# callmeray/PointMVSNet

Hardware: NVIDIA H100
Metric: PointFlow iters/sec (higher is better)
Workload: dtype f32

## Files before the change

### include/pmvs_b200.h

```cpp
#ifndef PMVS_B200_H_
#define PMVS_B200_H_

#include <stddef.h>
#include <stdint.h>

#ifdef __cplusplus
extern "C" {
#endif

#define PMVS_OK 0
#define PMVS_ERR_ARG 1
#define PMVS_ERR_CUDA 2
#define PMVS_ERR_WORKSPACE 3

#define PMVS_NUM_HYP 5
#define PMVS_FEAT_CH 136
#define PMVS_KNN 16
#define PMVS_MAX_VIEWS 12

typedef void* pmvs_stream_t;

int pmvs_version(void);
const char* pmvs_last_error(void);
unsigned long long pmvs_launch_count(void);

int pmvs_set_gemm_mode(int mode);
int pmvs_get_gemm_mode(void);

#define PMVS_OPT_EDGE 1
#define PMVS_OPT_KNN 2
#define PMVS_OPT_FETCH 3
#define PMVS_OPT_GEMM 4
#define PMVS_OPT_DEBUG_IDX 5
int pmvs_set_option(int key, int value);
int pmvs_get_option(int key);

int pmvs_profile_enable(int on);
int pmvs_profile_collect(char* names, size_t names_bytes, float* ms, int max_records);

int pmvs_gather_knn_forward(const float* input, const int64_t* index, float* output,
                            int B, int C, int N, int K, pmvs_stream_t stream);
int pmvs_gather_knn_backward(const float* grad_output, const int64_t* index, float* grad_input,
                             int B, int C, int N, int K, pmvs_stream_t stream);
size_t pmvs_gather_knn_backward_det_workspace_bytes(int B, int N, int K);
int pmvs_gather_knn_backward_det(const float* grad_output, const int64_t* index, float* grad_input,
                                 int B, int C, int N, int K, void* workspace, size_t workspace_bytes,
                                 pmvs_stream_t stream);

int pmvs_knn3d(const float* xyz, int64_t* idx64, int32_t* idx32, int B, int D, int H, int W,
               int ksize, int knn, pmvs_stream_t stream);

int pmvs_feature_fetch(const float* feature_maps, const float* pts, const float* intrinsics,
                       const float* extrinsics, float* out, int B, int V, int C, int H, int W,
                       int N, pmvs_stream_t stream);
int pmvs_feature_fetch_backward(const float* grad_out, const float* pts, const float* intrinsics,
                                const float* extrinsics, float* grad_maps, int B, int V, int C,
                                int H, int W, int N, pmvs_stream_t stream);

int pmvs_cost_volume(const float* features, const float* cam_params, float* cost, void* workspace,
                     size_t workspace_bytes, int B, int V, int C, int h, int w, int D, int is_test,
                     pmvs_stream_t stream);

int pmvs_transpose(const float* in, float* out, int batch, int R, int C, pmvs_stream_t stream);
int pmvs_idx64_to_idx32(const int64_t* in, int32_t* out, long long n, pmvs_stream_t stream);

int pmvs_edgeconv_pm(const float* x, int ldx, const int32_t* idx32, const float* w12,
                     const float* gamma, const float* beta, float eps, int concat_central,
                     int bn_train, float* out, int ldo, float* le_scratch, double* stats_scratch,
                     int groups, int rows_per_group, int N, int K, int cin, int cout,
                     pmvs_stream_t stream);

int pmvs_linear_pm(const float* x, int ldx, const float* w, float* y, int ldy, int groups,
                   int rows_per_group, int cin, int cout, const double* in_stats,
                   const float* in_gamma, const float* in_beta, double in_count, float eps,
                   double* out_stats, pmvs_stream_t stream);

typedef struct pmvs_flow_weights {
  const float* ec_w12[3];
  const float* ec_gamma[3];
  const float* ec_beta[3];
  const float* mlp_w[4];
  const float* mlp_gamma[3];
  const float* mlp_beta[3];
  float* ec_run_mean[3];
  float* ec_run_var[3];
  float* mlp_run_mean[3];
// ... 38 lines not shown
```

### pointmvsnet_b200/_lib.py

```python
import ctypes as C
import os

import torch

_HERE = os.path.dirname(os.path.abspath(__file__))
LIB_PATH = os.path.join(_HERE, "libpmvs_b200.so")

if not os.path.exists(LIB_PATH):
    raise ImportError(
        "pointmvsnet_b200: %s is missing -- build it with pointmvsnet_b200/csrc/build.sh "
        "(nvcc, sm_90a).  There is no CPU fallback." % LIB_PATH)

lib = C.CDLL(LIB_PATH)

c_float_p = C.c_void_p
c_stream = C.c_void_p


class FlowWeights(C.Structure):
    _fields_ = [
        ("ec_w12", C.c_void_p * 3), ("ec_gamma", C.c_void_p * 3), ("ec_beta", C.c_void_p * 3),
        ("mlp_w", C.c_void_p * 4), ("mlp_gamma", C.c_void_p * 3), ("mlp_beta", C.c_void_p * 3),
        ("ec_run_mean", C.c_void_p * 3), ("ec_run_var", C.c_void_p * 3),
        ("mlp_run_mean", C.c_void_p * 3), ("mlp_run_var", C.c_void_p * 3),
# ... 49 lines not shown
EXPORTED = [
    "pmvs_version", "pmvs_last_error", "pmvs_launch_count", "pmvs_set_option", "pmvs_get_option", "pmvs_profile_enable", "pmvs_profile_collect", "pmvs_set_gemm_mode", "pmvs_get_gemm_mode", "pmvs_gather_knn_forward",
    "pmvs_gather_knn_backward", "pmvs_gather_knn_backward_det_workspace_bytes", "pmvs_gather_knn_backward_det", "pmvs_knn3d", "pmvs_feature_fetch", "pmvs_feature_fetch_backward",
    "pmvs_cost_volume", "pmvs_transpose", "pmvs_idx64_to_idx32", "pmvs_edgeconv_pm", "pmvs_linear_pm", "pmvs_point_flow_workspace_bytes",
    "pmvs_point_flow_iter", "pmvs_pyramid_to_channels_last", "pmvs_point_flow_debug_offsets",
]


def check(rc):
    if rc != 0:
        raise RuntimeError("libpmvs_b200: " + lib.pmvs_last_error().decode("utf-8", "replace"))


def stream_ptr():
    return torch.cuda.current_stream().cuda_stream


def ptr(t):
    return None if t is None else t.data_ptr()


def require_cuda(*tensors):
    for t in tensors:
        if t is not None and not t.is_cuda:
            raise RuntimeError("pointmvsnet_b200 operators need CUDA tensors (sm_90a); there is no CPU fallback")


def f32c(t):
    if t.dtype != torch.float32:
        t = t.float()
    return t.contiguous()


def launch_count():
    return int(lib.pmvs_launch_count())


def profile_enable(on):
    lib.pmvs_profile_enable(1 if on else 0)


def profile_collect(max_records=65536):
    names = C.create_string_buffer(max_records * 24)
    ms = (C.c_float * max_records)()
    n = lib.pmvs_profile_collect(names, len(names), C.cast(ms, C.c_void_p), max_records)
    nm = names.value.decode().split("\n")[:n]
    return [(nm[i], float(ms[i])) for i in range(n)]


def set_gemm_mode(mode):
    check(lib.pmvs_set_gemm_mode(int(mode)))


OPTIONS = {"edge": 1, "knn": 2, "fetch": 3, "gemm": 4, "debug_idx": 5}


def set_option(name, value):
    check(lib.pmvs_set_option(OPTIONS[name], int(value)))


def get_option(name):
    return int(lib.pmvs_get_option(OPTIONS[name]))


def _options_from_env():
    spec = os.environ.get("PMVS_OPTIONS", "")
    for item in spec.split(","):
        if "=" in item:
            k, v = item.split("=", 1)
            set_option(k.strip(), int(v))


_options_from_env()
```

### pointmvsnet_b200/csrc/api.cu

```cuda
#include <algorithm>
#include <atomic>
#include <cstdarg>
#include <mutex>
#include <vector>

#include "common.cuh"

namespace pmvs {

static thread_local char g_err[512] = "";
static std::atomic<unsigned long long> g_launches{0};

void set_error(const char* fmt, ...) {
  va_list ap;
  va_start(ap, fmt);
  vsnprintf(g_err, sizeof(g_err), fmt, ap);
  va_end(ap);
}
void count_launch(int n) { g_launches.fetch_add((unsigned long long)n, std::memory_order_relaxed); }

static std::atomic<int> g_opt[OPT_COUNT];
static struct OptDefaults {
  OptDefaults() {
    g_opt[OPT_EDGE].store(1);
    g_opt[OPT_KNN].store(1);
    g_opt[OPT_FETCH].store(1);
    g_opt[OPT_GEMM].store(2);
  }
} g_opt_defaults;
int opt(int key) { return (key >= 0 && key < OPT_COUNT) ? g_opt[key].load(std::memory_order_relaxed) : 0; }

struct ProfRec {
  const char* name;
  cudaEvent_t a, b;
};
static std::mutex g_prof_mu;
static std::vector<ProfRec> g_prof;
static std::atomic<int> g_prof_on{0};
static thread_local int g_prof_open = -1;

void prof_begin(const char* what, cudaStream_t st) {
  if (!g_prof_on.load(std::memory_order_relaxed)) return;
  ProfRec r;
  r.name = what;
  if (cudaEventCreate(&r.a) != cudaSuccess || cudaEventCreate(&r.b) != cudaSuccess) return;
  cudaEventRecord(r.a, st);
  std::lock_guard<std::mutex> lk(g_prof_mu);
  g_prof.push_back(r);
  g_prof_open = (int)g_prof.size() - 1;
}
void prof_end(cudaStream_t st) {
  if (g_prof_open < 0) return;
  std::lock_guard<std::mutex> lk(g_prof_mu);
  if (g_prof_open < (int)g_prof.size()) cudaEventRecord(g_prof[g_prof_open].b, st);
  g_prof_open = -1;
}

__global__ void __launch_bounds__(256) transpose_kernel(const float* __restrict__ in, float* __restrict__ out, int R,
                                                        int C) {
  __shared__ float tile[32][33];
  const size_t boff = (size_t)blockIdx.z * R * C;
  const int c0 = blockIdx.x * 32, r0 = blockIdx.y * 32;
  const int tx = threadIdx.x & 31, ty = threadIdx.x >> 5;
#pragma unroll
  for (int j = 0; j < 32; j += 8) {
    const int r = r0 + ty + j, c = c0 + tx;
    if (r < R && c < C) tile[ty + j][tx] = __ldg(in + boff + (size_t)r * C + c);
  }
  __syncthreads();
#pragma unroll
  for (int j = 0; j < 32; j += 8) {
    const int c = c0 + ty + j, r = r0 + tx;
    if (r < R && c < C) out[boff + (size_t)c * R + r] = tile[tx][ty + j];
  }
}

int launch_transpose(const float* in, float* out, int batch, int R, int C, cudaStream_t st) {
  PMVS_REQUIRE(in && out && batch > 0 && R > 0 && C > 0, "transpose: bad arguments");
  PMVS_REQUIRE(batch <= 65535 && cdiv(R, 32) <= 65535, "transpose: shape too large");
  dim3 grid(cdiv(C, 32), cdiv(R, 32), batch);
// ... 393 lines not shown
```

### pointmvsnet_b200/csrc/common.cuh

```cuda
#pragma once
#include <cuda_runtime.h>
#include <stdint.h>
#include <stdio.h>
#include <string.h>

#include "../../include/pmvs_b200.h"

namespace pmvs {

void set_error(const char* fmt, ...);
void count_launch(int n = 1);

void prof_begin(const char* what, cudaStream_t st);
void prof_end(cudaStream_t st);

inline int check_launch(const char* what, cudaStream_t st = nullptr) {
  cudaError_t e = cudaPeekAtLastError();
  if (e != cudaSuccess) {
    cudaGetLastError();
    set_error("%s: %s", what, cudaGetErrorString(e));
    return PMVS_ERR_CUDA;
  }
  prof_end(st);
  count_launch();
  return PMVS_OK;
}

#define PMVS_REQUIRE(cond, ...)     \
  do {                              \
    if (!(cond)) {                  \
      pmvs::set_error(__VA_ARGS__); \
      return PMVS_ERR_ARG;          \
    }                               \
  } while (0)

#define PMVS_TRY(expr)           \
  do {                           \
    int _rc = (expr);            \
    if (_rc != PMVS_OK) return _rc; \
  } while (0)

static inline int cdiv(long long a, long long b) { return (int)((a + b - 1) / b); }

inline int sm_count() {
  static int n = 0;
  if (n == 0) {
    int dev = 0, v = 0;
    cudaGetDevice(&dev);
    n = (cudaDeviceGetAttribute(&v, cudaDevAttrMultiProcessorCount, dev) == cudaSuccess && v > 0) ? v : 132;
  }
  return n;
}

__device__ __forceinline__ float4 ldg4(const float* p) { return __ldg(reinterpret_cast<const float4*>(p)); }
__device__ __forceinline__ void st4(float* p, float4 v) { *reinterpret_cast<float4*>(p) = v; }

typedef float2 f32x2;
__device__ __forceinline__ f32x2 pack2(float a, float b) { return make_float2(a, b); }
__device__ __forceinline__ void unpack2(f32x2 v, float& a, float& b) { a = v.x; b = v.y; }
__device__ __forceinline__ f32x2 fma2(f32x2 a, f32x2 b, f32x2 c) { return make_float2(__fmaf_rn(a.x, b.x, c.x), __fmaf_rn(a.y, b.y, c.y)); }
__device__ __forceinline__ f32x2 add2(f32x2 a, f32x2 b) { return make_float2(__fadd_rn(a.x, b.x), __fadd_rn(a.y, b.y)); }
__device__ __forceinline__ f32x2 mul2(f32x2 a, f32x2 b) { return make_float2(__fmul_rn(a.x, b.x), __fmul_rn(a.y, b.y)); }
__device__ __forceinline__ f32x2 sub2(f32x2 a, f32x2 b) { return make_float2(__fsub_rn(a.x, b.x), __fsub_rn(a.y, b.y)); }

enum {
  OPT_EDGE = 1,
  OPT_KNN = 2,
  OPT_FETCH = 3,
  OPT_GEMM = 4,
  OPT_DEBUG_IDX = 5,
  OPT_COUNT = 16
};
int opt(int key);

template <typename K>
inline int ensure_dyn_smem(K kernel, int bytes, unsigned long long& done_mask, const char* what) {
  int dev = 0;
  if (cudaGetDevice(&dev) != cudaSuccess || dev < 0 || dev > 63) dev = 0;
  if (done_mask & (1ull << dev)) return PMVS_OK;
  if (cudaFuncSetAttribute(kernel, cudaFuncAttributeMaxDynamicSharedMemorySize, bytes) != cudaSuccess) {
    cudaGetLastError();
    set_error("%s: cannot reserve %d bytes of shared memory", what, bytes);
    return PMVS_ERR_CUDA;
  }
  done_mask |= 1ull << dev;
  return PMVS_OK;
}

struct BnCoef {
  float mean, invstd;
};
__device__ __forceinline__ BnCoef bn_coef(double s1, double s2, double count, float eps) {
  double m = s1 / count;
  double var = s2 / count - m * m;
  if (var < 0.0) var = 0.0;
  BnCoef c;
  c.mean = (float)m;
  c.invstd = (float)(1.0 / sqrt(var + (double)eps));
  return c;
}
__device__ __forceinline__ float bn_apply(float x, float mean, float invstd, float g, float b) {
  return __fadd_rn(__fmul_rn(__fmul_rn(__fsub_rn(x, mean), invstd), g), b);
}

int launch_knn3d_cand(const float* xyz, int32_t* idx32, unsigned short* cand, int clouds, int D, int H, int W,
                      cudaStream_t st);
int launch_knn3d(const float* xyz, int64_t* idx64, int32_t* idx32, int clouds, int D, int H, int W,
                 int ksize, int knn, cudaStream_t st);
int launch_transpose(const float* in, float* out, int batch, int R, int C, cudaStream_t st);

struct GemmArgs {
  const float* x;
  int ldx;
  const float* w;
  float* y;
  int ldy;
  int groups, rows_per_group, cin, cout;
  const double* in_stats;
  const float* in_gamma;
  const float* in_beta;
  double in_count;
  float eps;
  double* out_stats;
// ... 90 lines not shown
```

### pointmvsnet_b200/csrc/edge_tile.cu

```cuda
#include <algorithm>
#include <cuda.h>

#include "common.cuh"

namespace pmvs {

namespace {

constexpr int ET_THREADS = 256;
constexpr int ET_WARPS = ET_THREADS / 32;
constexpr int ET_CP = 32;
constexpr int ET_LPP = ET_CP / 4;
constexpr int ET_PPW = 32 / ET_LPP;

typedef CUresult (*EncodeTiledFn)(CUtensorMap*, CUtensorMapDataType, cuuint32_t, void*, const cuuint64_t*,
                                  const cuuint64_t*, const cuuint32_t*, const cuuint32_t*, CUtensorMapInterleave,
                                  CUtensorMapSwizzle, CUtensorMapL2promotion, CUtensorMapFloatOOBfill);

EncodeTiledFn encode_fn() {
  static EncodeTiledFn fn = [] {
    void* p = nullptr;
    cudaDriverEntryPointQueryResult q;
    if (cudaGetDriverEntryPoint("cuTensorMapEncodeTiled", &p, cudaEnableDefault, &q) != cudaSuccess ||
        q != cudaDriverEntryPointSuccess)
      p = nullptr;
    cudaGetLastError();
    return (EncodeTiledFn)p;
  }();
  return fn;
}

__device__ __forceinline__ unsigned smem_u32(const void* p) { return (unsigned)__cvta_generic_to_shared(p); }

template <int TX, int TY>
struct TileGeom {
  static constexpr int HX = TX + 4, HY = TY + 4;
  static constexpr int ROWS = PMVS_NUM_HYP * HY * HX;
  static constexpr int NPTS = PMVS_NUM_HYP * TY * TX;
  static constexpr int BYTES = ROWS * ET_CP * 4;
  static constexpr int SMEM = BYTES;
};

constexpr int ET_COEF = 6;

template <int COUT, bool APPLY, int TX, int TY>
__global__ void __launch_bounds__(ET_THREADS, 3) edge_tile_kernel(const __grid_constant__ CUtensorMap tm,
                                                                   const EdgeTileArgs a) {
  using G = TileGeom<TX, TY>;
  static_assert(COUT % ET_CP == 0, "edge_tile: channels must be a multiple of 32");
  static_assert(G::NPTS % (ET_WARPS * ET_PPW) == 0, "edge_tile: every thread owns NPTS / 32 points");
  constexpr int LD = 2 * COUT;
  constexpr int SLABS = COUT / ET_CP;
  constexpr int STEPS = G::NPTS / (ET_WARPS * ET_PPW);
  static_assert(G::HX == 12 && G::HY == 8, "the kNN kernel's 16-bit codes are row offsets of a 12 x 8 x 5 halo tile");
  extern __shared__ __align__(128) float halo[];
  __shared__ __align__(8) unsigned long long bar;
  __shared__ float part[APPLY ? 1 : ET_WARPS][APPLY ? 1 : 2 * ET_CP];
  __shared__ __align__(16) float coef[APPLY ? ET_COEF * COUT : 4];
  __shared__ int s_last;

  const int g = blockIdx.z;
  const int tid = threadIdx.x, warp = tid >> 5, lane = tid & 31;
  const int sub = lane / ET_LPP, cl = (lane % ET_LPP) * 4;
  const int gh = a.gh, gw = a.gw;
  const int tiles_x = (gw + TX - 1) / TX, tiles_per_cloud = tiles_x * ((gh + TY - 1) / TY);
  const int tiles_per_group = tiles_per_cloud * a.clouds_per_group;
  const int HW = gh * gw, N = PMVS_NUM_HYP * HW;
  const int rows_per_group = a.clouds_per_group * N;
  const unsigned bar_addr = smem_u32(&bar);

  if (tid == 0) {
    asm volatile("mbarrier.init.shared::cta.b64 [%0], 1;" ::"r"(bar_addr));
    asm volatile("fence.mbarrier_init.release.cluster;" ::: "memory");
  }
  if (APPLY) {
    const float* cg = a.coef + (size_t)g * ET_COEF * COUT;
    for (int c = tid; c < ET_COEF * COUT; c += ET_THREADS) coef[c] = __ldg(cg + c);
  }
  static_assert(TX * TY == ET_WARPS * ET_PPW && STEPS == PMVS_NUM_HYP, "edge_tile: one layer of the tile per step");
  const int tq = warp * ET_PPW + sub, tx = tq % TX, ty = tq / TX;
  const int pb0 = ((-2 * G::HY + ty) * G::HX + tx) * ET_CP + cl;
  constexpr int LAYER = G::HY * G::HX * ET_CP;
  __syncthreads();
// ... 138 lines not shown
      unpack2(n2_lo, v[4], v[5]); unpack2(n2_hi, v[6], v[7]);
#pragma unroll
      for (int off = ET_LPP; off < 32; off <<= 1) {
#pragma unroll
        for (int q = 0; q < 8; ++q) v[q] += __shfl_xor_sync(0xffffffffu, v[q], off);
      }
      if (sub == 0) {
#pragma unroll
        for (int q = 0; q < 8; ++q) part[warp][(q >> 2) * ET_CP + cl + (q & 3)] = v[q];
      }
      __syncthreads();
      double* o = a.nstats + (size_t)g * 2 * COUT;
      if (tid < 2 * ET_CP) {
        double t = 0.0;
#pragma unroll
        for (int wq = 0; wq < ET_WARPS; ++wq) t += (double)part[wq][tid];
        atomicAdd(o + (tid / ET_CP) * COUT + ch0 + (tid % ET_CP), t);
      }
    }
  }

  if (!APPLY) {
    __threadfence();
    __syncthreads();
    if (tid == 0) {
      const unsigned t = atomicAdd(a.ticket + g, 1u);
      s_last = t == gridDim.x - 1;
    }
    __syncthreads();
    if (s_last) {
      __threadfence();
      const double* sc = a.cstats + (size_t)g * 4 * COUT;
      const double* sn = a.nstats + (size_t)g * 2 * COUT;
      float* cg = a.coef + (size_t)g * ET_COEF * COUT;
      const double cnt_c = (double)rows_per_group, cnt_n = (double)rows_per_group * PMVS_KNN;
      for (int c = tid; c < COUT; c += ET_THREADS) {
        const BnCoef kn = bn_coef(__ldcg(sn + c), __ldcg(sn + COUT + c), cnt_n, a.eps);
        const int gn = a.concat_central ? COUT + c : c;
        const float A = kn.invstd * a.gamma[gn];
        cg[c] = A;
        cg[COUT + c] = fmaf(-kn.mean, A, a.beta[gn]);
        if (a.concat_central) {
          const BnCoef kc = bn_coef(sc[c], sc[2 * COUT + c], cnt_c, a.eps);
          cg[2 * COUT + c] = kc.mean; cg[3 * COUT + c] = kc.invstd; cg[4 * COUT + c] = a.gamma[c]; cg[5 * COUT + c] = a.beta[c];
        }
      }
    }
  }
}

template <int COUT, bool APPLY, int TX, int TY>
int launch_variant(const EdgeTileArgs& a, cudaStream_t st) {
  using G = TileGeom<TX, TY>;
  EncodeTiledFn enc = encode_fn();
  if (enc == nullptr) {
    set_error("edge_tile: cuTensorMapEncodeTiled is not available from this driver");
    return PMVS_ERR_CUDA;
  }
  const int N = PMVS_NUM_HYP * a.gh * a.gw;
  const long long layers = (long long)a.groups * a.clouds_per_group * PMVS_NUM_HYP;
  PMVS_REQUIRE(a.groups <= 65535 && a.clouds_per_group <= 65535, "edge_tile: too many clouds");
  PMVS_REQUIRE(layers < (1ll << 31) && (long long)a.groups * a.clouds_per_group * N < (1ll << 40), "edge_tile: too large");
  PMVS_REQUIRE(((uintptr_t)a.le & 15) == 0, "edge_tile: LE must be 16-byte aligned");
  CUtensorMap tm;
  const cuuint64_t gdim[4] = {(cuuint64_t)(2 * COUT), (cuuint64_t)a.gw, (cuuint64_t)a.gh, (cuuint64_t)layers};
  const cuuint64_t gstr[3] = {(cuuint64_t)(2 * COUT) * 4, (cuuint64_t)a.gw * 2 * COUT * 4,
                              (cuuint64_t)a.gh * a.gw * 2 * COUT * 4};
  const cuuint32_t box[4] = {ET_CP, (cuuint32_t)G::HX, (cuuint32_t)G::HY, PMVS_NUM_HYP};
  const cuuint32_t estr[4] = {1, 1, 1, 1};
  const CUresult r = enc(&tm, CU_TENSOR_MAP_DATA_TYPE_FLOAT32, 4, const_cast<float*>(a.le), gdim, gstr, box, estr,
                         CU_TENSOR_MAP_INTERLEAVE_NONE, CU_TENSOR_MAP_SWIZZLE_NONE, CU_TENSOR_MAP_L2_PROMOTION_L2_128B,
                         CU_TENSOR_MAP_FLOAT_OOB_FILL_NONE);
  if (r != CUDA_SUCCESS) {
    set_error("edge_tile: cuTensorMapEncodeTiled failed (%d) for %dx%d, cout %d", (int)r, a.gh, a.gw, COUT);
    return PMVS_ERR_CUDA;
  }
  static unsigned long long smem_done = 0;
  PMVS_TRY(ensure_dyn_smem(edge_tile_kernel<COUT, APPLY, TX, TY>, G::SMEM, smem_done, "edge_tile"));
  static int slots = 0;
  if (slots == 0) {
    slots = 3 * sm_count();
  }
  const int tiles_per_group = cdiv(a.gw, TX) * cdiv(a.gh, TY) * a.clouds_per_group;
  int ctas = APPLY ? tiles_per_group : std::min(tiles_per_group, std::max(1, slots / a.groups));
  ctas = cdiv(tiles_per_group, cdiv(tiles_per_group, ctas));
  PMVS_REQUIRE(ctas <= 0x7fffffff / 2, "edge_tile: too many tiles");
  dim3 grid(ctas, 1, a.groups);
  static const char* const names[2][2] = {{"edge_stats_32", "edge_stats_64"}, {"edge_apply_32", "edge_apply_64"}};
  prof_begin(names[APPLY ? 1 : 0][COUT == 32 ? 0 : 1], st);
  edge_tile_kernel<COUT, APPLY, TX, TY><<<grid, ET_THREADS, G::SMEM, st>>>(tm, a);
  return check_launch(APPLY ? "edge_tile_apply_kernel" : "edge_tile_stats_kernel", st);
}

template <bool APPLY>
int launch_edge_tile(const EdgeTileArgs& a, int tile_w, cudaStream_t st) {
  PMVS_REQUIRE(a.le && a.cand && a.cstats && a.nstats && a.gamma && a.beta && a.coef && a.ticket && (!APPLY || a.out),
               "edge_tile: NULL pointer");
  PMVS_REQUIRE(a.cout == 32 || a.cout == 64, "edge_tile: out_channels %d (supported: 32, 64)", a.cout);
  PMVS_REQUIRE(a.gh > 0 && a.gw > 0 && a.groups > 0 && a.clouds_per_group > 0, "edge_tile: bad cloud shape");
  (void)tile_w;
  return a.cout == 32 ? launch_variant<32, APPLY, 8, 4>(a, st) : launch_variant<64, APPLY, 8, 4>(a, st);
}

}

int launch_edge_tile_stats(const EdgeTileArgs& a, int tile_w, cudaStream_t st) {
  return launch_edge_tile<false>(a, tile_w, st);
// ... 7 lines not shown
```

### pointmvsnet_b200/csrc/gemm_ws.cu

```cuda
#include <algorithm>

#include "common.cuh"
#include "wgmma.cuh"

namespace pmvs {

namespace ws {

using namespace wg;

constexpr int NT = 128;
constexpr int KC = 32;
constexpr int PLANE_BYTES = NT * KC * 4;
constexpr int STAGE_BYTES = 2 * PLANE_BYTES;
constexpr int CONS_WARPS = 8, CONS_THREADS = CONS_WARPS * 32;
constexpr int PROD_WARPS = 8, PROD_WARP0 = CONS_WARPS, PROD_THREADS = PROD_WARPS * 32;
constexpr int THREADS = CONS_THREADS + PROD_THREADS;
constexpr int A_LD = NT * 8 / PROD_THREADS;
static_assert(A_LD * PROD_THREADS == NT * 8, "the producers share a chunk evenly");
constexpr int MAXK = 224;
constexpr int SMEM_MAX = 227 * 1024;

template <int ASYNC, int NSTAGES>
struct Layout {
  static constexpr int NST = NSTAGES;
  static constexpr int RING = 0;
  static constexpr int STAGING = RING + NST * STAGE_BYTES;
  static constexpr int W = STAGING + ASYNC * PLANE_BYTES;
};
__host__ __device__ constexpr int weight_bytes(int cout, int nch) { return nch * 2 * cout * 128; }
constexpr int TAIL_BN = 0, TAIL_RED = TAIL_BN + 2 * MAXK * 4;
__host__ __device__ constexpr int tail_bar(int cout) { return TAIL_RED + 2 * cout * 8; }
__host__ __device__ constexpr int tail_bytes(int cout) { return tail_bar(cout) + 128; }

__device__ __forceinline__ void sts128(uint32_t addr, float4 v) {
  asm volatile("st.shared.v4.f32 [%0], {%1, %2, %3, %4};" ::"r"(addr), "f"(v.x), "f"(v.y), "f"(v.z), "f"(v.w) : "memory");
}
__device__ __forceinline__ float4 lds128(uint32_t addr) {
  float4 v;
  asm volatile("ld.shared.v4.f32 {%0, %1, %2, %3}, [%4];" : "=f"(v.x), "=f"(v.y), "=f"(v.z), "=f"(v.w) : "r"(addr) : "memory");
  return v;
}
__device__ __forceinline__ float tf32_hi(float x) { return __uint_as_float(__float_as_uint(x) & 0xFFFFE000u); }

struct TileRange {
  int first, count;
};
__device__ __forceinline__ TileRange my_tiles(int total) {
  const long long G = gridDim.x, b = blockIdx.x;
  const int lo = (int)(b * total / G), hi = (int)((b + 1) * total / G);
  return TileRange{lo, hi - lo};
}

template <int COUT, bool IN_BN, int ASYNC, int NSTAGES>
__global__ void __launch_bounds__(THREADS, 1) gemm_ws_kernel(const GemmArgs a) {
// ... 247 lines not shown
          if (!ok1) v[2] = v[3] = 0.f;
          float s[4] = {v[0] + v[2], v[1] + v[3], fmaf(v[0], v[0], v[2] * v[2]), fmaf(v[1], v[1], v[3] * v[3])};
#pragma unroll
          for (int e = 0; e < 4; ++e) {
            s[e] += __shfl_xor_sync(0xffffffffu, s[e], 4);
            s[e] += __shfl_xor_sync(0xffffffffu, s[e], 8);
            s[e] += __shfl_xor_sync(0xffffffffu, s[e], 16);
          }
          if (lane < 4) {
            atomicAdd(&sRed[8 * i + fcol], (double)s[0]);
            atomicAdd(&sRed[8 * i + fcol + 1], (double)s[1]);
            atomicAdd(&sRed[COUT + 8 * i + fcol], (double)s[2]);
            atomicAdd(&sRed[COUT + 8 * i + fcol + 1], (double)s[3]);
          }
        }
      }
      if (a.out_stats != nullptr) {
        named_bar_sync(2, CONS_THREADS);
        if (tid < 2 * COUT) {
          racc += sRed[tid];
          sRed[tid] = 0.0;
        }
        named_bar_sync(2, CONS_THREADS);
      }
    }
    flush();
  }
}

constexpr int DEEP_K = 160;
template <int ASYNC, int NSTAGES>
constexpr int smem_bytes(int cout, int cin) {
  return Layout<ASYNC, NSTAGES>::W + weight_bytes(cout, (cin + KC - 1) / KC) + tail_bytes(cout);
}
constexpr bool fits(int cin, int cout) {
  return cin <= DEEP_K ? (smem_bytes<4, 2>(cout, cin) <= SMEM_MAX && smem_bytes<0, 4>(cout, cin) <= SMEM_MAX)
                       : (smem_bytes<3, 2>(cout, cin) <= SMEM_MAX && smem_bytes<0, 3>(cout, cin) <= SMEM_MAX);
}
static_assert(fits(136, 64) && fits(32, 64) && fits(64, 128) && fits(224, 64) && fits(64, 64) && fits(64, 16),
              "a hot-path GEMM shape no longer fits the shared memory of gemm_ws_kernel");

template <int COUT, bool IN_BN, int ASYNC, int NSTAGES>
static int launch_pf(const GemmArgs& a, cudaStream_t st, const char* name) {
  const int smem_total = smem_bytes<ASYNC, NSTAGES>(COUT, a.cin);
  if (smem_total > SMEM_MAX) return -1;
  static unsigned long long smem_done = 0;
  PMVS_TRY((ensure_dyn_smem(gemm_ws_kernel<COUT, IN_BN, ASYNC, NSTAGES>, SMEM_MAX, smem_done, "gemm_ws")));
  const long long tiles = (long long)a.groups * cdiv(a.rows_per_group, NT);
  const int grid = (int)std::min<long long>(tiles, sm_count());
  prof_begin(name, st);
  gemm_ws_kernel<COUT, IN_BN, ASYNC, NSTAGES><<<grid, THREADS, smem_total, st>>>(a);
  return check_launch("gemm_ws_kernel", st);
}
template <int COUT, bool IN_BN>
static int launch_one(const GemmArgs& a, cudaStream_t st, const char* name) {
  const bool deep = a.cin <= DEEP_K;
  if (opt(OPT_GEMM) == 1)
    return deep ? launch_pf<COUT, IN_BN, 0, 4>(a, st, name) : launch_pf<COUT, IN_BN, 0, 3>(a, st, name);
  return deep ? launch_pf<COUT, IN_BN, 4, 2>(a, st, name) : launch_pf<COUT, IN_BN, 3, 2>(a, st, name);
}

}

int launch_gemm_ws(const GemmArgs& a, cudaStream_t st, const char* name) {
  if (a.cin % 8 != 0 || a.cin > ws::MAXK || a.ldx % 4 != 0 || a.ldy % 2 != 0 || a.groups <= 0 || a.rows_per_group <= 0) return -1;
  if (((uintptr_t)a.x & 15) || ((uintptr_t)a.w & 15) || ((uintptr_t)a.y & 7)) return -1;
  if ((long long)a.groups * cdiv(a.rows_per_group, ws::NT) >= (1ll << 31) / ws::MAXK) return -1;
  const bool bn = a.in_stats != nullptr;
  switch (a.cout) {
    case 16: return bn ? ws::launch_one<16, true>(a, st, name) : ws::launch_one<16, false>(a, st, name);
    case 32: return bn ? ws::launch_one<32, true>(a, st, name) : ws::launch_one<32, false>(a, st, name);
    case 64: return bn ? ws::launch_one<64, true>(a, st, name) : ws::launch_one<64, false>(a, st, name);
    case 128: return bn ? ws::launch_one<128, true>(a, st, name) : ws::launch_one<128, false>(a, st, name);
  }
  return -1;
}

}
```

### pointmvsnet_b200/csrc/wgmma.cuh

```cuda
#pragma once
#include <stdint.h>

namespace pmvs {
namespace wg {

__device__ __forceinline__ uint32_t smem_u32(const void* p) { return (uint32_t)__cvta_generic_to_shared(p); }
__device__ __forceinline__ void mbar_init(uint32_t bar, uint32_t count) {
  asm volatile("mbarrier.init.shared::cta.b64 [%0], %1;" ::"r"(bar), "r"(count));
}
__device__ __forceinline__ void mbar_wait(uint32_t bar, uint32_t parity) {
  uint32_t done = 0;
  while (!done) {
    asm volatile(
        "{\n\t.reg .pred p;\n\t"
        "mbarrier.try_wait.parity.shared::cta.b64 p, [%1], %2;\n\t"
        "selp.u32 %0, 1, 0, p;\n\t}"
        : "=r"(done)
        : "r"(bar), "r"(parity)
        : "memory");
  }
}
__device__ __forceinline__ void mbar_arrive(uint32_t bar) {
  asm volatile("mbarrier.arrive.shared::cta.b64 _, [%0];" ::"r"(bar) : "memory");
}
__device__ __forceinline__ void fence_proxy_async() { asm volatile("fence.proxy.async.shared::cta;" ::: "memory"); }
__device__ __forceinline__ void named_bar_sync(int id, int nthreads) {
  asm volatile("bar.sync %0, %1;" ::"r"(id), "r"(nthreads) : "memory");
}

__device__ __forceinline__ int swz128(int r, int pc) { return (r >> 3) * 1024 + (r & 7) * 128 + ((pc ^ (r & 7)) << 4); }

__device__ __forceinline__ uint64_t make_desc(uint32_t smem_addr) {
  return (uint64_t)((smem_addr >> 4) & 0x3FFF) | ((uint64_t)1 << 16) | ((uint64_t)(1024 >> 4) << 32) | ((uint64_t)1 << 62);
}

__device__ __forceinline__ void fence() { asm volatile("wgmma.fence.sync.aligned;" ::: "memory"); }
__device__ __forceinline__ void commit() { asm volatile("wgmma.commit_group.sync.aligned;" ::: "memory"); }
__device__ __forceinline__ void wait_all() { asm volatile("wgmma.wait_group.sync.aligned 0;" ::: "memory"); }
template <int R>
__device__ __forceinline__ void fence_regs(float (&d)[R]) {
#pragma unroll
  for (int i = 0; i < R; ++i) asm volatile("" : "+f"(d[i])::"memory");
}

template <int N>
__device__ __forceinline__ void mma_tf32(float* d, uint64_t adesc, uint64_t bdesc, uint32_t accumulate);
template <>
__device__ __forceinline__ void mma_tf32<16>(float* d, uint64_t adesc, uint64_t bdesc, uint32_t accumulate) {
  asm volatile(
      "{\n\t.reg .pred p;\n\tsetp.ne.b32 p, %10, 0;\n\t"
      "wgmma.mma_async.sync.aligned.m64n16k8.f32.tf32.tf32 {"
      "%0, %1, %2, %3, %4, %5, %6, %7}, "
      "%8, %9, p, 1, 1;\n\t}"
      : "+f"(d[0]), "+f"(d[1]), "+f"(d[2]), "+f"(d[3]), "+f"(d[4]), "+f"(d[5]),
        "+f"(d[6]), "+f"(d[7])
      : "l"(adesc), "l"(bdesc), "r"(accumulate));
}
template <>
__device__ __forceinline__ void mma_tf32<32>(float* d, uint64_t adesc, uint64_t bdesc, uint32_t accumulate) {
  asm volatile(
      "{\n\t.reg .pred p;\n\tsetp.ne.b32 p, %18, 0;\n\t"
      "wgmma.mma_async.sync.aligned.m64n32k8.f32.tf32.tf32 {"
      "%0, %1, %2, %3, %4, %5, %6, %7, %8, %9, %10, %11, %12, %13, %14, %15}, "
      "%16, %17, p, 1, 1;\n\t}"
      : "+f"(d[0]), "+f"(d[1]), "+f"(d[2]), "+f"(d[3]), "+f"(d[4]), "+f"(d[5]),
        "+f"(d[6]), "+f"(d[7]), "+f"(d[8]), "+f"(d[9]), "+f"(d[10]), "+f"(d[11]),
        "+f"(d[12]), "+f"(d[13]), "+f"(d[14]), "+f"(d[15])
      : "l"(adesc), "l"(bdesc), "r"(accumulate));
}
template <>
__device__ __forceinline__ void mma_tf32<64>(float* d, uint64_t adesc, uint64_t bdesc, uint32_t accumulate) {
  asm volatile(
      "{\n\t.reg .pred p;\n\tsetp.ne.b32 p, %34, 0;\n\t"
      "wgmma.mma_async.sync.aligned.m64n64k8.f32.tf32.tf32 {"
      "%0, %1, %2, %3, %4, %5, %6, %7, %8, %9, %10, %11, %12, %13, %14, %15, "
      "%16, %17, %18, %19, %20, %21, %22, %23, %24, %25, %26, %27, %28, %29, %30, %31}, "
      "%32, %33, p, 1, 1;\n\t}"
      : "+f"(d[0]), "+f"(d[1]), "+f"(d[2]), "+f"(d[3]), "+f"(d[4]), "+f"(d[5]),
        "+f"(d[6]), "+f"(d[7]), "+f"(d[8]), "+f"(d[9]), "+f"(d[10]), "+f"(d[11]),
        "+f"(d[12]), "+f"(d[13]), "+f"(d[14]), "+f"(d[15]), "+f"(d[16]), "+f"(d[17]),
        "+f"(d[18]), "+f"(d[19]), "+f"(d[20]), "+f"(d[21]), "+f"(d[22]), "+f"(d[23]),
        "+f"(d[24]), "+f"(d[25]), "+f"(d[26]), "+f"(d[27]), "+f"(d[28]), "+f"(d[29]),
        "+f"(d[30]), "+f"(d[31])
      : "l"(adesc), "l"(bdesc), "r"(accumulate));
}

template <int N, int BLK>
__device__ __forceinline__ void mma_tile(float* d, uint32_t a_addr, uint32_t b_addr, uint32_t accumulate) {
  static_assert(N % BLK == 0 && (BLK == 16 || BLK == 32 || BLK == 64), "block shape");
#pragma unroll
  for (int nb = 0; nb < N / BLK; ++nb)
    mma_tf32<BLK>(d + (BLK / 2) * nb, make_desc(a_addr), make_desc(b_addr + nb * BLK * 128), accumulate);
}

}
}
```

Measured before the change: 1155.

## Add TMA-fed warp-specialized GEMM with register-A wgmma and make it default

```diff
diff --git a/include/pmvs_b200.h b/include/pmvs_b200.h
--- a/include/pmvs_b200.h
+++ b/include/pmvs_b200.h
@@ -32,6 +32,7 @@
 #define PMVS_OPT_FETCH 3
 #define PMVS_OPT_GEMM 4
 #define PMVS_OPT_DEBUG_IDX 5
+#define PMVS_OPT_GEMM_STRICT 6
 int pmvs_set_option(int key, int value);
 int pmvs_get_option(int key);
 
diff --git a/pointmvsnet_b200/_lib.py b/pointmvsnet_b200/_lib.py
--- a/pointmvsnet_b200/_lib.py
+++ b/pointmvsnet_b200/_lib.py
@@ -125,7 +125,7 @@
     check(lib.pmvs_set_gemm_mode(int(mode)))
 
 
-OPTIONS = {"edge": 1, "knn": 2, "fetch": 3, "gemm": 4, "debug_idx": 5}
+OPTIONS = {"edge": 1, "knn": 2, "fetch": 3, "gemm": 4, "debug_idx": 5, "gemm_strict": 6}
 
 
 def set_option(name, value):
diff --git a/pointmvsnet_b200/csrc/api.cu b/pointmvsnet_b200/csrc/api.cu
--- a/pointmvsnet_b200/csrc/api.cu
+++ b/pointmvsnet_b200/csrc/api.cu
@@ -25,7 +25,7 @@
     g_opt[OPT_EDGE].store(1);
     g_opt[OPT_KNN].store(1);
     g_opt[OPT_FETCH].store(1);
-    g_opt[OPT_GEMM].store(2);
+    g_opt[OPT_GEMM].store(3);
   }
 } g_opt_defaults;
 int opt(int key) { return (key >= 0 && key < OPT_COUNT) ? g_opt[key].load(std::memory_order_relaxed) : 0; }
diff --git a/pointmvsnet_b200/csrc/common.cuh b/pointmvsnet_b200/csrc/common.cuh
--- a/pointmvsnet_b200/csrc/common.cuh
+++ b/pointmvsnet_b200/csrc/common.cuh
@@ -69,6 +69,7 @@
   OPT_FETCH = 3,
   OPT_GEMM = 4,
   OPT_DEBUG_IDX = 5,
+  OPT_GEMM_STRICT = 6,
   OPT_COUNT = 16
 };
 int opt(int key);
diff --git a/pointmvsnet_b200/csrc/edge_tile.cu b/pointmvsnet_b200/csrc/edge_tile.cu
--- a/pointmvsnet_b200/csrc/edge_tile.cu
+++ b/pointmvsnet_b200/csrc/edge_tile.cu
@@ -1,7 +1,7 @@
 #include <algorithm>
-#include <cuda.h>
 
 #include "common.cuh"
+#include "tensor_map.cuh"
 
 namespace pmvs {
 
@@ -12,23 +12,6 @@
 constexpr int ET_CP = 32;
 constexpr int ET_LPP = ET_CP / 4;
 constexpr int ET_PPW = 32 / ET_LPP;
-
-typedef CUresult (*EncodeTiledFn)(CUtensorMap*, CUtensorMapDataType, cuuint32_t, void*, const cuuint64_t*,
-                                  const cuuint64_t*, const cuuint32_t*, const cuuint32_t*, CUtensorMapInterleave,
-                                  CUtensorMapSwizzle, CUtensorMapL2promotion, CUtensorMapFloatOOBfill);
-
-EncodeTiledFn encode_fn() {
-  static EncodeTiledFn fn = [] {
-    void* p = nullptr;
-    cudaDriverEntryPointQueryResult q;
-    if (cudaGetDriverEntryPoint("cuTensorMapEncodeTiled", &p, cudaEnableDefault, &q) != cudaSuccess ||
-        q != cudaDriverEntryPointSuccess)
-      p = nullptr;
-    cudaGetLastError();
-    return (EncodeTiledFn)p;
-  }();
-  return fn;
-}
 
 __device__ __forceinline__ unsigned smem_u32(const void* p) { return (unsigned)__cvta_generic_to_shared(p); }
 
@@ -273,7 +256,7 @@
 template <int COUT, bool APPLY, int TX, int TY>
 int launch_variant(const EdgeTileArgs& a, cudaStream_t st) {
   using G = TileGeom<TX, TY>;
-  EncodeTiledFn enc = encode_fn();
+  EncodeTiledFn enc = encode_tiled_fn();
   if (enc == nullptr) {
     set_error("edge_tile: cuTensorMapEncodeTiled is not available from this driver");
     return PMVS_ERR_CUDA;
diff --git a/pointmvsnet_b200/csrc/gemm_ws.cu b/pointmvsnet_b200/csrc/gemm_ws.cu
--- a/pointmvsnet_b200/csrc/gemm_ws.cu
+++ b/pointmvsnet_b200/csrc/gemm_ws.cu
@@ -1,6 +1,8 @@
 #include <algorithm>
+#include <type_traits>
 
 #include "common.cuh"
+#include "tensor_map.cuh"
 #include "wgmma.cuh"
 
 namespace pmvs {
@@ -354,8 +356,304 @@
   gemm_ws_kernel<COUT, IN_BN, ASYNC, NSTAGES><<<grid, THREADS, smem_total, st>>>(a);
   return check_launch("gemm_ws_kernel", st);
 }
+namespace tma {
+constexpr int NT = 64;
+constexpr int STAGE_BYTES = NT * KC * 4;
+constexpr int CONS_THREADS = 256;
+constexpr int THREADS = CONS_THREADS + 64;
+constexpr int MAX_STAGES = 32, MIN_STAGES = 8;
+constexpr int BN_FLOATS = (MAXK / KC) * 4 * 16;
+constexpr int TAIL_BN = 0, TAIL_RED = TAIL_BN + 2 * BN_FLOATS * 4;
+__host__ __device__ constexpr int tail_bar(int cout) { return TAIL_RED + 2 * 2 * cout * 8; }
+__host__ __device__ constexpr int tail_bytes(int cout) { return tail_bar(cout) + 2 * MAX_STAGES * 8; }
+__host__ __device__ constexpr int stages_for(int cin, int cout) {
+  return (SMEM_MAX - weight_bytes(cout, (cin + KC - 1) / KC) - tail_bytes(cout)) / STAGE_BYTES < MAX_STAGES
+             ? (SMEM_MAX - weight_bytes(cout, (cin + KC - 1) / KC) - tail_bytes(cout)) / STAGE_BYTES
+             : MAX_STAGES;
+}
+}
+
+template <int N>
+__device__ __forceinline__ void reduce_scatter_round(float* sv, int lane, int m) {
+  const bool up = (lane & m) != 0;
+#pragma unroll
+  for (int k = 0; k < N / 2; ++k) {
+    const float keep = up ? sv[k + N / 2] : sv[k], send = up ? sv[k] : sv[k + N / 2];
+    sv[k] = keep + __shfl_xor_sync(0xffffffffu, send, m);
+  }
+}
+
+template <int COUT, bool IN_BN>
+__global__ void __launch_bounds__(tma::THREADS, 1) gemm_tma_kernel(const __grid_constant__ CUtensorMap tmx,
+                                                                   const GemmArgs a, const int wstages) {
+  constexpr int NT = tma::NT, STAGE_BYTES = tma::STAGE_BYTES, CONS_THREADS = tma::CONS_THREADS;
+  constexpr int MAX_STAGES = tma::MAX_STAGES, BN_FLOATS = tma::BN_FLOATS, TAIL_BN = tma::TAIL_BN, TAIL_RED = tma::TAIL_RED;
+  constexpr bool STACKED = COUT <= 64;
+  constexpr int W_CHUNK = 2 * COUT * 128;
+  constexpr int ACC_REGS = (STACKED ? 2 * COUT : COUT) / 2;
+  constexpr int BLK = COUT < 64 ? COUT : 64;
+  extern __shared__ __align__(1024) unsigned char smem[];
+  const uint32_t smem_base = smem_u32(smem);
+
+  const int K = a.cin;
+  const int nch = (K + KC - 1) / KC;
+  const int tid = threadIdx.x, warp = __shfl_sync(0xffffffffu, tid >> 5, 0), lane = tid & 31;
+  const int tpg = (a.rows_per_group + NT - 1) / NT;
+  const TileRange tr = my_tiles(a.groups * tpg);
+  unsigned char* tail = smem + weight_bytes(COUT, nch) + 2 * wstages * STAGE_BYTES;
+  const uint32_t bar0 = smem_u32(tail + tma::tail_bar(COUT));
+  auto bar_full = [&](int w, int s) { return bar0 + 8u * (uint32_t)(w * (MAX_STAGES / 2) + s); };
+  auto bar_empty = [&](int w, int s) { return bar0 + 8u * (uint32_t)(MAX_STAGES + w * (MAX_STAGES / 2) + s); };
+
+  if (tid == 0) {
+    for (int w = 0; w < 2; ++w)
+      for (int s = 0; s < wstages; ++s) {
+        mbar_init(bar_full(w, s), 1);
+        mbar_init(bar_empty(w, s), 4);
+      }
+    asm volatile("fence.mbarrier_init.release.cluster;" ::: "memory");
+  }
+  __syncthreads();
+
+  if (warp >= CONS_THREADS / 32) {
+    const int w = warp - CONS_THREADS / 32;
+    if (lane == 0) {
+      const uint32_t ring = smem_base + weight_bytes(COUT, nch) + w * wstages * STAGE_BYTES;
+      int stage = 0;
+      uint32_t phase = 0;
+      for (int i = w; i < tr.count; i += 2) {
+        const int t = tr.first + i, g = t / tpg, row0 = (t - g * tpg) * NT;
+        for (int c = 0; c < nch; ++c) {
+          mbar_wait(bar_empty(w, stage), phase ^ 1u);
+          mbar_arrive_expect_tx(bar_full(w, stage), STAGE_BYTES);
+          tma_load_3d(ring + stage * STAGE_BYTES, &tmx, c * KC, row0, g, bar_full(w, stage));
+          if (++stage == wstages) {
+            stage = 0;
+            phase ^= 1u;
+          }
+        }
+      }
+    }
+    return;
+  }
+
+  const int wgi = warp >> 2, wtid = tid & 127;
+  const uint32_t ring = smem_base + weight_bytes(COUT, nch) + wgi * wstages * STAGE_BYTES;
+  float* sBN = (float*)(tail + TAIL_BN) + wgi * BN_FLOATS;
+  double* sRed = (double*)(tail + TAIL_RED) + wgi * 2 * COUT;
+  for (int i = wtid; i < 2 * COUT; i += 128) sRed[i] = 0.0;
+  for (int e = tid; e < COUT * nch * 8; e += CONS_THREADS) {
+    const int n = e / (nch * 8), rem = e - n * (nch * 8), c = rem >> 3, pc = rem & 7;
+    const int k0 = c * KC + pc * 4;
+    const float4 v = k0 < K ? ldg4(a.w + (size_t)n * K + k0) : make_float4(0.f, 0.f, 0.f, 0.f);
+    float4 hi, lo;
+    hi.x = tf32_hi(v.x); hi.y = tf32_hi(v.y); hi.z = tf32_hi(v.z); hi.w = tf32_hi(v.w);
+    lo.x = __fsub_rn(v.x, hi.x); lo.y = __fsub_rn(v.y, hi.y); lo.z = __fsub_rn(v.z, hi.z); lo.w = __fsub_rn(v.w, hi.w);
+    const uint32_t dst = smem_base + c * W_CHUNK + swz128(n, pc);
+    sts128(dst, hi);
+    sts128(dst + COUT * 128, lo);
+  }
+  fence_proxy_async();
+  named_bar_sync(1, CONS_THREADS);
+
+  const int r = (warp & 3) * 16 + (lane >> 2), q = lane & 3;
+  const uint32_t fbase = r * 128 + q * 4, fx = (r & 7) << 4;
+  const int frow = r, fcol = 2 * q;
+  const uint32_t w_base = smem_base;
+  float acc[ACC_REGS];
+  uint32_t fh[16], fl[16];
+  const uint32_t wg_bar = 2 + wgi;
+
+  constexpr int HC = COUT < 64 ? COUT : 64, NH = COUT / HC;
+  constexpr int NV = HC / 16;
+  const int kofs = ((lane >> 2) & 1) * (8 * NV / 2) + ((lane >> 3) & 1) * (8 * NV / 4) + ((lane >> 4) & 1) * (8 * NV / 8);
+  double racc[NH][NV];
+#pragma unroll
+  for (int h = 0; h < NH; ++h)
+#pragma unroll
+    for (int j = 0; j < NV; ++j) racc[h][j] = 0.0;
+  auto flush = [&](int g) {
+    if (a.out_stats == nullptr) return;
+#pragma unroll
+    for (int h = 0; h < NH; ++h)
+#pragma unroll
+      for (int j = 0; j < NV; ++j) {
+        const int k = kofs + j, i = (k >> 2) + h * (HC / 8), e = k & 3;
+        atomicAdd(&sRed[(e >> 1) * COUT + 8 * i + fcol + (e & 1)], racc[h][j]);
+        racc[h][j] = 0.0;
+      }
+    named_bar_sync(wg_bar, 128);
+    for (int s = wtid; s < 2 * COUT; s += 128) {
+      atomicAdd(a.out_stats + (size_t)g * 2 * a.cout + s, sRed[s]);
+      sRed[s] = 0.0;
+    }
+  };
+
+  auto chunk = [&](auto KSTEPS, int c, int m) {
+    constexpr int ksteps = decltype(KSTEPS)::value;
+    const int stage = m % wstages;
+    mbar_wait(bar_full(wgi, stage), (uint32_t)((m / wstages) & 1));
+    const uint32_t st = ring + stage * STAGE_BYTES + fbase;
+    float bA[8], bB[8];
+    if (IN_BN) {
+      const float4* t4 = reinterpret_cast<const float4*>(sBN + (c * 4 + q) * 16);
+      const float4 a0 = t4[0], a1 = t4[1], b0 = t4[2], b1 = t4[3];
+      bA[0] = a0.x; bA[1] = a0.y; bA[2] = a0.z; bA[3] = a0.w; bA[4] = a1.x; bA[5] = a1.y; bA[6] = a1.z; bA[7] = a1.w;
+      bB[0] = b0.x; bB[1] = b0.y; bB[2] = b0.z; bB[3] = b0.w; bB[4] = b1.x; bB[5] = b1.y; bB[6] = b1.z; bB[7] = b1.w;
+    }
+#pragma unroll
+    for (int j = 0; j < 4; ++j) {
+      if (j < ksteps) {
+#pragma unroll
+        for (int h = 0; h < 2; ++h) {
+          const uint32_t addr = st + ((uint32_t)((2 * j + h) << 4) ^ fx);
+          float v[2];
+          asm volatile("ld.shared.f32 %0, [%1];" : "=f"(v[0]) : "r"(addr) : "memory");
+          asm volatile("ld.shared.f32 %0, [%1];" : "=f"(v[1]) : "r"(addr + 1024) : "memory");
+#pragma unroll
+          for (int e = 0; e < 2; ++e) {
+            float x = v[e];
+            if (IN_BN) x = fmaxf(fmaf(x, bA[2 * j + h], bB[2 * j + h]), 0.f);
+            const float hi = tf32_hi(x);
+            fh[4 * j + 2 * h + e] = __float_as_uint(hi);
+            fl[4 * j + 2 * h + e] = __float_as_uint(__fsub_rn(x, hi));
+          }
+        }
+      }
+    }
+    fence();
+    const uint32_t w_hi = w_base + c * W_CHUNK, w_lo = w_hi + COUT * 128;
+#pragma unroll
+    for (int j = 0; j < 4; ++j) {
+      if (j < ksteps) {
+        const uint32_t first = (c | j) != 0 ? 1u : 0u;
+        if (STACKED) {
+          mma_tile_ra<2 * COUT, BLK>(acc, &fh[4 * j], w_hi + j * 32, first);
+          mma_tile_ra<COUT, BLK>(acc + COUT / 2, &fl[4 * j], w_hi + j * 32, 1u);
+        } else {
+          mma_tile_ra<COUT, BLK>(acc, &fl[4 * j], w_hi + j * 32, first);
+          mma_tile_ra<COUT, BLK>(acc, &fh[4 * j], w_lo + j * 32, 1u);
+          mma_tile_ra<COUT, BLK>(acc, &fh[4 * j], w_hi + j * 32, 1u);
+        }
+      }
+    }
+    commit();
+    wait<0>();
+    fence_regs(fh);
+    fence_regs(fl);
+    __syncwarp();
+    if (lane == 0) mbar_arrive(bar_empty(wgi, stage));
+  };
+  auto chunk_ks = [&](int c, int m) {
+    switch (min(KC, K - c * KC) / 8) {
+      case 4: chunk(std::integral_constant<int, 4>(), c, m); break;
+      case 3: chunk(std::integral_constant<int, 3>(), c, m); break;
+      case 2: chunk(std::integral_constant<int, 2>(), c, m); break;
+      default: chunk(std::integral_constant<int, 1>(), c, m); break;
+    }
+  };
+
+  int cur_g = -1;
+  for (int i = wgi; i < tr.count; i += 2) {
+    const int t = tr.first + i;
+    const int g = t / tpg, row0 = (t - g * tpg) * NT;
+    const int rows_valid = min(NT, a.rows_per_group - row0);
+    const size_t grow0 = (size_t)g * a.rows_per_group + row0;
+    if (g != cur_g) {
+      named_bar_sync(wg_bar, 128);
+      if (cur_g >= 0) flush(cur_g);
+      if (IN_BN) {
+        const double* s = a.in_stats + (size_t)g * 2 * K;
+        for (int e = wtid; e < nch * 64; e += 128) {
+          const int c = e >> 6, qq = (e >> 4) & 3, k = e & 15, jh = k & 7;
+          const int col = c * KC + 8 * (jh >> 1) + qq + 4 * (jh & 1);
+          float val = 0.f;
+          if (col < K) {
+            const BnCoef bc = bn_coef(s[col], s[K + col], a.in_count, a.eps);
+            const float A = __fmul_rn(bc.invstd, a.in_gamma[col]);
+            val = k < 8 ? A : fmaf(-bc.mean, A, a.in_beta[col]);
+          }
+          sBN[e] = val;
+        }
+      }
+      named_bar_sync(wg_bar, 128);
+      cur_g = g;
+    }
+    const int m0 = (i >> 1) * nch;
+    for (int c = 0; c < nch; ++c) chunk_ks(c, m0 + c);
+    fence_regs(acc);
+    const bool ok0 = frow < rows_valid, ok1 = frow + 8 < rows_valid;
+    float* y0 = a.y + (grow0 + frow) * a.ldy + fcol;
+    float* y1 = y0 + (size_t)8 * a.ldy;
+#pragma unroll
+    for (int h = 0; h < NH; ++h) {
+      float sv[HC / 2];
+#pragma unroll
+      for (int il = 0; il < HC / 8; ++il) {
+        const int ii = h * (HC / 8) + il;
+        float v[4];
+#pragma unroll
+        for (int e = 0; e < 4; ++e) v[e] = STACKED ? acc[4 * ii + e] + acc[COUT / 2 + 4 * ii + e] : acc[4 * ii + e];
+        if (ok0) *reinterpret_cast<float2*>(y0 + 8 * ii) = make_float2(v[0], v[1]);
+        if (ok1) *reinterpret_cast<float2*>(y1 + 8 * ii) = make_float2(v[2], v[3]);
+        if (!ok0) v[0] = v[1] = 0.f;
+        if (!ok1) v[2] = v[3] = 0.f;
+        sv[4 * il + 0] = v[0] + v[2];
+        sv[4 * il + 1] = v[1] + v[3];
+        sv[4 * il + 2] = fmaf(v[0], v[0], v[2] * v[2]);
+        sv[4 * il + 3] = fmaf(v[1], v[1], v[3] * v[3]);
+      }
+      if (a.out_stats != nullptr) {
+        reduce_scatter_round<HC / 2>(sv, lane, 4);
+        reduce_scatter_round<HC / 4>(sv, lane, 8);
+        reduce_scatter_round<HC / 8>(sv, lane, 16);
+#pragma unroll
+        for (int j = 0; j < NV; ++j) racc[h][j] += (double)sv[j];
+      }
+    }
+  }
+  if (cur_g >= 0) flush(cur_g);
+}
+
+static_assert(tma::stages_for(136, 64) >= tma::MIN_STAGES && tma::stages_for(32, 64) >= tma::MIN_STAGES &&
+                  tma::stages_for(64, 128) >= tma::MIN_STAGES && tma::stages_for(224, 64) >= tma::MIN_STAGES &&
+                  tma::stages_for(64, 64) >= tma::MIN_STAGES && tma::stages_for(64, 16) >= tma::MIN_STAGES,
+              "a hot-path GEMM shape no longer gets the minimum ring depth of gemm_tma_kernel");
+
+template <int COUT, bool IN_BN>
+static int launch_tma(const GemmArgs& a, cudaStream_t st, const char* name) {
+  const int stages = tma::stages_for(a.cin, COUT);
+  if (stages < tma::MIN_STAGES) return -1;
+  const int wstages = stages / 2;
+  const unsigned long long row_bytes = (unsigned long long)a.ldx * 4, group_bytes = row_bytes * a.rows_per_group;
+  if (group_bytes >= (1ull << 40) || (unsigned long long)a.groups > 0xffffffffull) return -1;
+  EncodeTiledFn enc = encode_tiled_fn();
+  if (enc == nullptr) return -1;
+  CUtensorMap tm;
+  const cuuint64_t gdim[3] = {(cuuint64_t)a.cin, (cuuint64_t)a.rows_per_group, (cuuint64_t)a.groups};
+  const cuuint64_t gstr[2] = {row_bytes, group_bytes};
+  const cuuint32_t box[3] = {KC, tma::NT, 1};
+  const cuuint32_t estr[3] = {1, 1, 1};
+  if (enc(&tm, CU_TENSOR_MAP_DATA_TYPE_FLOAT32, 3, const_cast<float*>(a.x), gdim, gstr, box, estr,
+          CU_TENSOR_MAP_INTERLEAVE_NONE, CU_TENSOR_MAP_SWIZZLE_128B, CU_TENSOR_MAP_L2_PROMOTION_L2_256B,
+          CU_TENSOR_MAP_FLOAT_OOB_FILL_NONE) != CUDA_SUCCESS)
+    return -1;
+  const int smem_total = weight_bytes(COUT, cdiv(a.cin, KC)) + 2 * wstages * tma::STAGE_BYTES + tma::tail_bytes(COUT);
+  static unsigned long long smem_done = 0;
+  PMVS_TRY((ensure_dyn_smem(gemm_tma_kernel<COUT, IN_BN>, SMEM_MAX, smem_done, "gemm_tma")));
+  const long long tiles = (long long)a.groups * cdiv(a.rows_per_group, tma::NT);
+  const int grid = (int)std::min<long long>(tiles, sm_count());
+  prof_begin(name, st);
+  gemm_tma_kernel<COUT, IN_BN><<<grid, tma::THREADS, smem_total, st>>>(tm, a, wstages);
+  return check_launch("gemm_tma_kernel", st);
+}
+
 template <int COUT, bool IN_BN>
 static int launch_one(const GemmArgs& a, cudaStream_t st, const char* name) {
+  if (opt(OPT_GEMM) == 3) {
+    const int rc = launch_tma<COUT, IN_BN>(a, st, name);
+    if (rc >= 0 || opt(OPT_GEMM_STRICT)) return rc;
+  }
   const bool deep = a.cin <= DEEP_K;
   if (opt(OPT_GEMM) == 1)
     return deep ? launch_pf<COUT, IN_BN, 0, 4>(a, st, name) : launch_pf<COUT, IN_BN, 0, 3>(a, st, name);
@@ -364,7 +662,7 @@
 
 }
 
-int launch_gemm_ws(const GemmArgs& a, cudaStream_t st, const char* name) {
+static int launch_gemm_ws_any(const GemmArgs& a, cudaStream_t st, const char* name) {
   if (a.cin % 8 != 0 || a.cin > ws::MAXK || a.ldx % 4 != 0 || a.ldy % 2 != 0 || a.groups <= 0 || a.rows_per_group <= 0) return -1;
   if (((uintptr_t)a.x & 15) || ((uintptr_t)a.w & 15) || ((uintptr_t)a.y & 7)) return -1;
   if ((long long)a.groups * cdiv(a.rows_per_group, ws::NT) >= (1ll << 31) / ws::MAXK) return -1;
@@ -378,4 +676,14 @@
   return -1;
 }
 
-}
+int launch_gemm_ws(const GemmArgs& a, cudaStream_t st, const char* name) {
+  const int rc = launch_gemm_ws_any(a, st, name);
+  if (rc < 0 && opt(OPT_GEMM) == 3 && opt(OPT_GEMM_STRICT)) {
+    set_error("gemm: gemm_tma_kernel does not take cin %d, cout %d, ldx %d, %d groups of %d rows (strict mode)", a.cin,
+              a.cout, a.ldx, a.groups, a.rows_per_group);
+    return PMVS_ERR_ARG;
+  }
+  return rc;
+}
+
+}
diff --git a/pointmvsnet_b200/csrc/tensor_map.cuh b/pointmvsnet_b200/csrc/tensor_map.cuh
--- /dev/null
+++ b/pointmvsnet_b200/csrc/tensor_map.cuh
@@ -0,0 +1,24 @@
+#pragma once
+#include <cuda.h>
+#include <cuda_runtime.h>
+
+namespace pmvs {
+
+typedef CUresult (*EncodeTiledFn)(CUtensorMap*, CUtensorMapDataType, cuuint32_t, void*, const cuuint64_t*,
+                                  const cuuint64_t*, const cuuint32_t*, const cuuint32_t*, CUtensorMapInterleave,
+                                  CUtensorMapSwizzle, CUtensorMapL2promotion, CUtensorMapFloatOOBfill);
+
+inline EncodeTiledFn encode_tiled_fn() {
+  static EncodeTiledFn fn = [] {
+    void* p = nullptr;
+    cudaDriverEntryPointQueryResult q;
+    if (cudaGetDriverEntryPoint("cuTensorMapEncodeTiled", &p, cudaEnableDefault, &q) != cudaSuccess ||
+        q != cudaDriverEntryPointSuccess)
+      p = nullptr;
+    cudaGetLastError();
+    return (EncodeTiledFn)p;
+  }();
+  return fn;
+}
+
+}
diff --git a/pointmvsnet_b200/csrc/wgmma.cuh b/pointmvsnet_b200/csrc/wgmma.cuh
--- a/pointmvsnet_b200/csrc/wgmma.cuh
+++ b/pointmvsnet_b200/csrc/wgmma.cuh
@@ -26,6 +26,15 @@
 __device__ __forceinline__ void fence_proxy_async() { asm volatile("fence.proxy.async.shared::cta;" ::: "memory"); }
 __device__ __forceinline__ void named_bar_sync(int id, int nthreads) {
   asm volatile("bar.sync %0, %1;" ::"r"(id), "r"(nthreads) : "memory");
+}
+__device__ __forceinline__ void mbar_arrive_expect_tx(uint32_t bar, uint32_t bytes) {
+  asm volatile("mbarrier.arrive.expect_tx.shared::cta.b64 _, [%0], %1;" ::"r"(bar), "r"(bytes) : "memory");
+}
+__device__ __forceinline__ void tma_load_3d(uint32_t dst, const void* tmap, int c0, int c1, int c2, uint32_t bar) {
+  asm volatile(
+      "cp.async.bulk.tensor.3d.shared::cluster.global.mbarrier::complete_tx::bytes [%0], [%1, {%2, %3, %4}], [%5];"
+      ::"r"(dst), "l"(tmap), "r"(c0), "r"(c1), "r"(c2), "r"(bar)
+      : "memory");
 }
 
 __device__ __forceinline__ int swz128(int r, int pc) { return (r >> 3) * 1024 + (r & 7) * 128 + ((pc ^ (r & 7)) << 4); }
@@ -93,5 +102,61 @@
     mma_tf32<BLK>(d + (BLK / 2) * nb, make_desc(a_addr), make_desc(b_addr + nb * BLK * 128), accumulate);
 }
 
+template <int N>
+__device__ __forceinline__ void wait() { asm volatile("wgmma.wait_group.sync.aligned %0;" ::"n"(N) : "memory"); }
+template <int R>
+__device__ __forceinline__ void fence_regs(uint32_t (&d)[R]) {
+#pragma unroll
+  for (int i = 0; i < R; ++i) asm volatile("" : "+r"(d[i])::"memory");
+}
+
+template <int N>
+__device__ __forceinline__ void mma_tf32_ra(float* d, const uint32_t* a, uint64_t bdesc, uint32_t accumulate);
+template <>
+__device__ __forceinline__ void mma_tf32_ra<16>(float* d, const uint32_t* a, uint64_t bdesc, uint32_t accumulate) {
+  asm volatile(
+      "{\n\t.reg .pred p;\n\tsetp.ne.b32 p, %13, 0;\n\t"
+      "wgmma.mma_async.sync.aligned.m64n16k8.f32.tf32.tf32 {"
+      "%0, %1, %2, %3, %4, %5, %6, %7}, "
+      "{%8, %9, %10, %11}, %12, p, 1, 1;\n\t}"
+      : "+f"(d[0]), "+f"(d[1]), "+f"(d[2]), "+f"(d[3]), "+f"(d[4]), "+f"(d[5]),
+        "+f"(d[6]), "+f"(d[7])
+      : "r"(a[0]), "r"(a[1]), "r"(a[2]), "r"(a[3]), "l"(bdesc), "r"(accumulate));
+}
+template <>
+__device__ __forceinline__ void mma_tf32_ra<32>(float* d, const uint32_t* a, uint64_t bdesc, uint32_t accumulate) {
+  asm volatile(
+      "{\n\t.reg .pred p;\n\tsetp.ne.b32 p, %21, 0;\n\t"
+      "wgmma.mma_async.sync.aligned.m64n32k8.f32.tf32.tf32 {"
+      "%0, %1, %2, %3, %4, %5, %6, %7, %8, %9, %10, %11, %12, %13, %14, %15}, "
+      "{%16, %17, %18, %19}, %20, p, 1, 1;\n\t}"
+      : "+f"(d[0]), "+f"(d[1]), "+f"(d[2]), "+f"(d[3]), "+f"(d[4]), "+f"(d[5]),
+        "+f"(d[6]), "+f"(d[7]), "+f"(d[8]), "+f"(d[9]), "+f"(d[10]), "+f"(d[11]),
+        "+f"(d[12]), "+f"(d[13]), "+f"(d[14]), "+f"(d[15])
+      : "r"(a[0]), "r"(a[1]), "r"(a[2]), "r"(a[3]), "l"(bdesc), "r"(accumulate));
+}
+template <>
+__device__ __forceinline__ void mma_tf32_ra<64>(float* d, const uint32_t* a, uint64_t bdesc, uint32_t accumulate) {
+  asm volatile(
+      "{\n\t.reg .pred p;\n\tsetp.ne.b32 p, %37, 0;\n\t"
+      "wgmma.mma_async.sync.aligned.m64n64k8.f32.tf32.tf32 {"
+      "%0, %1, %2, %3, %4, %5, %6, %7, %8, %9, %10, %11, %12, %13, %14, %15, "
+      "%16, %17, %18, %19, %20, %21, %22, %23, %24, %25, %26, %27, %28, %29, %30, %31}, "
+      "{%32, %33, %34, %35}, %36, p, 1, 1;\n\t}"
+      : "+f"(d[0]), "+f"(d[1]), "+f"(d[2]), "+f"(d[3]), "+f"(d[4]), "+f"(d[5]),
+        "+f"(d[6]), "+f"(d[7]), "+f"(d[8]), "+f"(d[9]), "+f"(d[10]), "+f"(d[11]),
+        "+f"(d[12]), "+f"(d[13]), "+f"(d[14]), "+f"(d[15]), "+f"(d[16]), "+f"(d[17]),
+        "+f"(d[18]), "+f"(d[19]), "+f"(d[20]), "+f"(d[21]), "+f"(d[22]), "+f"(d[23]),
+        "+f"(d[24]), "+f"(d[25]), "+f"(d[26]), "+f"(d[27]), "+f"(d[28]), "+f"(d[29]),
+        "+f"(d[30]), "+f"(d[31])
+      : "r"(a[0]), "r"(a[1]), "r"(a[2]), "r"(a[3]), "l"(bdesc), "r"(accumulate));
+}
+template <int N, int BLK>
+__device__ __forceinline__ void mma_tile_ra(float* d, const uint32_t* a, uint32_t b_addr, uint32_t accumulate) {
+  static_assert(N % BLK == 0 && (BLK == 16 || BLK == 32 || BLK == 64), "block shape");
+#pragma unroll
+  for (int nb = 0; nb < N / BLK; ++nb) mma_tf32_ra<BLK>(d + (BLK / 2) * nb, a, make_desc(b_addr + nb * BLK * 128), accumulate);
+}
+
 }
 }
```

Result: faster. 1374 (median of 6 runs) (+19.0%).
